# kris927b/TextBlaster

Measured on AMD Instinct MI355X. Metric: documents/sec through full C4+Gopher+langID pipeline at 1/2/4/8 MI355X, higher is better.
Workload: dtype bf16

## Files before the change

### csrc/common/docproc.h

```cpp
#pragma once
#include <type_traits>

#include "devplan.h"
#include "hash.h"
#include "langid.h"
#include "par.h"
#include "uax29.h"
#include "ucd.h"

namespace tb {

enum : int {
  PH_START = 0, PH_DECODE, PH_DICT, PH_PREFIX_HASH, PH_WORDS, PH_LINES, PH_GQ, PH_GR_LINES, PH_GR_WORDS,
  PH_GR_TOP, PH_GR_DUP, PH_FW, PH_LID, PH_GR_DUP_WALK, PH_GR_DUP_CANON, PH_GR_TOP_CANON,
  PH_C4_LOREM = 16, PH_C4_DECODE, PH_C4_LINES, PH_C4_CITE, PH_C4_WORDS, PH_C4_CODES, PH_C4_JOIN, PH_C4_SENT,
  PH_GR_NL = 24, PH_GR_LINE_DUP, PH_GR_WH, PH_GR_WCANON, PH_GQ_WORDS, PH_GQ_BYTES, PH_RUST_LINES,
  kPhaseSlots = 32
};

enum : uint32_t {
  DOC_OK = 0,
  DOC_NEEDS_CPU = 1,
  DOC_OVERFLOW = 2,
};
// ... 1246 lines not shown
    x.par.single([&]() {
      ex->rs = rs; ex->rl = rl; ex->prs = prs; ex->off = off; ex->ph = ph;
      ex->NR = NR; ex->NPR = NPR; ex->tcs = tcs; ex->tce = tce;
      ex->lines_valid = split_lines ? 1u : 0u;
    });
  }
  x.stamp(PH_GR_LINES);
  x.par.single([&]() {
    r[0] = span;
    r[1] = NPR + 1;
    r[2] = para_dup;
    r[3] = para_dup_b;
    r[4] = NR + 1;
    r[5] = line_dup;
    r[6] = line_dup_b;
  });
  const uint32_t W = w.n;
  const bool ngrams = ds.n_top + ds.n_dup > 0;
  if constexpr (P::kWaves == 1) {
    if (ngrams && W >= kWave16) {
      x.set_flag(DOC_NEEDS_CPU);
      return;
    }
  }
  uint32_t* wid = nullptr;
  uint32_t* WL = nullptr;
  uint64_t* K = nullptr;
  uint64_t* PB = nullptr;
  if (ngrams && pre && pre->wready) {
    wid = pre->wid;
    WL = pre->wl;
    K = pre->wk;
    PB = pre->wpb;
  } else if (ngrams) {
    const uint64_t tab_bytes = 6ull * W + 64;
    wid = ex ? x.template alloc<uint32_t>(W + 1) : x.template alloc_hot_keep<uint32_t>(W + 1, tab_bytes);
    WL = ex ? x.template alloc<uint32_t>(W + 1) : x.template alloc_hot_keep<uint32_t>(W + 1, tab_bytes);
    K = ex ? x.template alloc<uint64_t>(W + 1) : x.template alloc_hot_keep<uint64_t>(W + 1, tab_bytes);
    PB = ex ? x.template alloc<uint64_t>(W + 1) : x.template alloc_hot_keep<uint64_t>(W + 1, tab_bytes);
    const bool early = P::kWaves == 1 && release_props && ex != nullptr;
    const auto mw = x.mark();
    uint64_t* wh = early ? x.template alloc_hot<uint64_t>(W + 1) : x.template alloc_hot_hi<uint64_t>(W + 1);
    if (x.overflow) return;
    x.par.for_n(W, [&](uint32_t k) { wh[k] = span_hash8(x, ph, w.bs[k], w.be[k]); });
    x.par.sync();
    if (early) x.release_hi();
    x.stamp(PH_GR_WH);
    canonicalize(
        x, W, [&](uint32_t k) { return dev_key(wh[k], w.be[k] - w.bs[k]); },
        [&](uint32_t i, uint32_t j) { return bytes_eq<P>(b, w.bs[i], w.be[i], w.bs[j], w.be[j]); }, wid);
    x.stamp(PH_GR_WCANON);
    const uint32_t totl = x.par.template scan<uint32_t>(
        W, 0u, [](uint32_t a, uint32_t c2) { return a + c2; },
        [&](uint32_t k) { return w.be[k] - w.bs[k]; }, [&](uint32_t k, uint32_t e) { WL[k] = e; });
    x.par.single([&]() { WL[W] = totl; });
    x.par.sync();
    x.par.for_n(W + 1, [&](uint32_t k) { PB[k] = x.powb(WL[k]); });
    const uint64_t ktot = x.par.template scan<uint64_t>(
        W, 0ull, [](uint64_t a, uint64_t c2) { return a + c2; },
        [&](uint32_t j) { return wh[j] * x.ipowb(WL[j + 1]); }, [&](uint32_t k, uint64_t e) { K[k] = e; });
    x.par.single([&]() { K[W] = ktot; });
    x.par.sync();
    x.reset(mw);
    if (x.overflow) return;
  }
  x.stamp(PH_GR_WORDS);
  if (release_props) x.release_hi();
  if (ngrams) {
    const DupGrams dg{wid, WL, K, PB, w.bs, w.be, b};
// ... 1415 lines not shown
```

### csrc/hip/kernels.hip

```cpp
#include <hip/hip_runtime.h>
#include <algorithm>
#include <cstdlib>
#include <string>

#include "../common/docproc.h"
#include "../common/gate.h"
#include "../common/badwords.h"

using namespace tb;

namespace {

constexpr uint32_t kMaxLdsPerDoc = 160 * 1024;
constexpr uint32_t kMaxLdsPerBlk = 128 * 1024;

struct DevTables {
  const uint16_t* s1;
  const uint32_t* s2;
  const uint16_t* l1;
  const int32_t* l2;
};

extern __shared__ __attribute__((aligned(16))) char g_lds_arena[];

// ... 146 lines not shown
    x.prof = nullptr;
    x.lds = lds_bytes ? (char*)g_lds_arena : nullptr;
    x.lcap = lds_bytes;
    x.lused = 0;
    x.ucd = UcdView{tabs.s1, tabs.s2, tabs.l1, tabs.l2};
    x.pw = pw;
    x.pw_n = pw_n;
    x.ipw = pw ? pw + pw_n + 1 : nullptr;
    const uint64_t region = (e.free_cap / (uint64_t)n_tasks) & ~255ull;
    x.scr = e.free_base + (uint64_t)t * region;
    x.cap = region;
    x.used = 0;
    x.flag = flags + doc;
    x.par.xs = g_block_xs;
    int64_t* r = rec + (int64_t)ds.rec_prefix * ndocs + (int64_t)doc * ds.width;
    if (t < ds.n_dup) gr_dup_one_order(x, ds, t, e, r);
    else if (t < ds.n_dup + ds.n_top) gr_top_one_order(x, ds, t - ds.n_dup, e, r);
    else if (t < ds.n_dup + ds.n_top + 2) gr_lines_split(x, t - ds.n_dup - ds.n_top, e, r);
    if (x.overflow) x.set_flag(DOC_NEEDS_CPU | DOC_OVERFLOW);
    __syncthreads();
  }
}

constexpr int kNgWaves = 4;

template <uint32_t MAXW>
struct NgShared {
  static_assert(MAXW % 64 == 0, "whole waves of grams");
  static constexpr uint32_t kMaxW = MAXW;
  static constexpr uint32_t kCap = MAXW + MAXW / 2 + 4;
  static constexpr uint32_t kSW = (MAXW + 31) / 32 + 1;
  static constexpr uint32_t kBW = MAXW / 2;
  static_assert(2 * kBW <= kCap && (kBW & (kBW - 1)) == 0, "bitmaps fit the table space");
  static constexpr uint32_t kDupBytes = 4 * kCap + 3 * 2 * MAXW + 4 * 2 * ((kSW + 3) & ~3u);
  static constexpr uint32_t kTopBytes = 4 * kCap + 2 * MAXW + 4 * MAXW;
  static constexpr uint32_t kRegion = ((kDupBytes > kTopBytes ? kDupBytes : kTopBytes) + 15) & ~15u;
  uint64_t K[MAXW + 1];
  uint64_t PB[MAXW + 1];
  uint16_t wid[MAXW + 1];
  uint16_t WL[MAXW + 1];
  uint4 region[kNgWaves][kRegion / 16];
};

__device__ __forceinline__ bool ng_fits(const GrExport& e, uint32_t hi) {
  return e.W <= hi && e.WL[e.W] <= 0xFFFFu;
}

__device__ __forceinline__ uint32_t ng_home(uint64_t k, uint32_t capn) {
  return (uint32_t)(((k & 0xFFFFFFFFull) * capn) >> 32);
}

template <class NS, class KeyF>
__device__ __forceinline__ uint32_t ng_candidates(uint32_t G, uint32_t lane, uint32_t* once, uint32_t* twice,
                                                  uint16_t* hbuf, uint16_t* list, KeyF&& key) {
  constexpr uint32_t kMask = NS::kBW * 32u - 1u;
  static_assert(kMask <= 0xFFFFu, "bit index in 16 bits");
#pragma unroll 1
  for (uint32_t p = lane; p < G; p += 64) {
    const uint32_t h = (uint32_t)(key(p) >> 20) & kMask;
    hbuf[p] = (uint16_t)h;
    const uint32_t bit = 1u << (h & 31u);
    if (atomicOr(&once[h >> 5], bit) & bit) atomicOr(&twice[h >> 5], bit);
  }
  __builtin_amdgcn_wave_barrier();
  const uint64_t lt = lane ? (~0ull >> (64 - lane)) : 0ull;
  uint32_t nc = 0;
#pragma unroll 1
  for (uint32_t base = 0; base < G; base += 64) {
    const uint32_t p = base + lane;
    bool c = false;
    if (p < G) {
      const uint32_t h = hbuf[p];
      c = (twice[h >> 5] >> (h & 31u)) & 1u;
    }
    const uint64_t m = __ballot(c);
    if (c) list[nc + (uint32_t)__popcll(m & lt)] = (uint16_t)p;
    nc += (uint32_t)__popcll(m);
  }
  __builtin_amdgcn_wave_barrier();
  return nc;
}

__device__ __attribute__((noinline)) bool ng_dup_eq_bytes(const GrExport* ep, uint32_t p, uint32_t q, uint32_t n) {
  const DupGrams dg{ep->wid, ep->WL, ep->K, ep->PB, ep->bs, ep->be, ep->b};
  return dg.eq(p, q, n);
}
template <class NS>
__device__ __forceinline__ bool ng_dup_eq(const NS& S, const GrExport* ep, uint32_t p, uint32_t q, uint32_t n) {
  if ((uint32_t)(S.WL[p + n] - S.WL[p]) != (uint32_t)(S.WL[q + n] - S.WL[q])) return false;
  uint32_t dw = 0;
  for (uint32_t k = 0; k < n; ++k) dw |= (uint32_t)(S.wid[p + k] ^ S.wid[q + k]);
  if (dw == 0) return true;
  return ng_dup_eq_bytes(ep, p, q, n);
}

template <class NS>
__device__ __forceinline__ int64_t ng_dup_order(NS& S, const GrExport* ep, uint32_t W, uint32_t n, uint32_t lane,
                                                uint4* region, bool prof, uint64_t& c_canon, uint64_t& c_walk) {
  const uint64_t t0 = prof ? __builtin_amdgcn_s_memtime() : 0;
  const uint32_t G = W - n + 1;
  const uint32_t SW = (G + 31) / 32 + 1;
  const uint32_t SWa = (SW + 3u) & ~3u;
  uint32_t* tab = (uint32_t*)region;
  uint16_t* gc = (uint16_t*)(tab + NS::kCap);
  uint16_t* list = gc + NS::kMaxW;
  uint16_t* gsl = list + NS::kMaxW;
  uint32_t* sn = (uint32_t*)(gsl + NS::kMaxW);
  uint32_t* R = sn + SWa;
  for (uint32_t i = lane; i < 2 * NS::kBW; i += 64) tab[i] = 0;
  for (uint32_t i = lane; i < 2 * SWa; i += 64) sn[i] = 0;
  __builtin_amdgcn_wave_barrier();
  auto key = [&](uint32_t p) {
    return dev_key(S.PB[p + n] * (S.K[p + n] - S.K[p]), (uint32_t)(S.WL[p + n] - S.WL[p]));
  };
  const uint32_t nc = ng_candidates<NS>(G, lane, tab, tab + NS::kBW, gc, list, key);
  if (nc < 2) {
    if (prof) c_canon += __builtin_amdgcn_s_memtime() - t0;
    return 0;
  }
  const uint32_t capn = nc + (nc >> 1) + 2;
  for (uint32_t i = lane; i < capn; i += 64) tab[i] = 0;
  __builtin_amdgcn_wave_barrier();
#pragma unroll 1
  for (uint32_t c = lane; c < nc; c += 64) {
    const uint32_t p = list[c];
    const uint64_t k = key(p);
    const uint32_t fp = (uint32_t)(k >> 48);
    const uint32_t mine = (fp << 16) | (c + 1);
    uint32_t sl = ng_home(k, capn);
    while (true) {
      uint32_t cur = tab[sl];
      if (cur == 0) {
        cur = atomicCAS(&tab[sl], 0u, mine);
        if (cur == 0) break;
      }
      if ((cur >> 16) == fp && ng_dup_eq(S, ep, p, list[(cur & 0xFFFFu) - 1u], n)) {
        if ((cur & 0xFFFFu) > c + 1u) atomicMin(&tab[sl], mine);
        break;
      }
      if (++sl == capn) sl = 0;
    }
    gsl[c] = (uint16_t)sl;
  }
  __builtin_amdgcn_wave_barrier();
#pragma unroll 1
  for (uint32_t c = lane; c < nc; c += 64) {
    const uint32_t g = (tab[gsl[c]] & 0xFFFFu) - 1u;
    const uint32_t p = list[c];
    gc[p] = (uint16_t)g;
    if (g != c) {
// ... 45 lines not shown
        A &= A - 1;
      }
    }
    if ((fv >> lane) & 1ull) atomicOr(&sn[g >> 5], 1u << (g & 31));
    uint32_t add = ((cnt >> lane) & 1ull) ? l : 0u;
    for (int o = 32; o > 0; o >>= 1) add += (uint32_t)__shfl_xor((int)add, o);
    rep += add;
    __builtin_amdgcn_wave_barrier();
    idx = next;
  }
  if (prof) c_walk += __builtin_amdgcn_s_memtime() - t1;
  return rep;
}

template <class NS>
__device__ __forceinline__ int64_t ng_top_order(NS& S, uint32_t W, uint32_t n, uint32_t lane, uint4* region) {
  const uint32_t G = W - n + 1;
  uint32_t* tab = (uint32_t*)region;
  uint16_t* list = (uint16_t*)(tab + NS::kCap);
  uint32_t* cnt = (uint32_t*)(list + NS::kMaxW);
  for (uint32_t i = lane; i < 2 * NS::kBW; i += 64) tab[i] = 0;
  __builtin_amdgcn_wave_barrier();
  auto key = [&](uint32_t p) {
    uint64_t h = (uint64_t)n << 56;
    for (uint32_t k = 0; k < n; ++k) h = (h ^ S.wid[p + k]) * 0x9E3779B97F4A7C15ull + k;
    return mix64(h);
  };
  const uint32_t nc = ng_candidates<NS>(G, lane, tab, tab + NS::kBW, (uint16_t*)cnt, list, key);
  if (nc < 2) return 0;
  const uint32_t capn = nc + (nc >> 1) + 2;
  for (uint32_t i = lane; i < capn; i += 64) tab[i] = 0;
  __builtin_amdgcn_wave_barrier();
#pragma unroll 1
  for (uint32_t c = lane; c < nc; c += 64) {
    const uint32_t p = list[c];
    const uint64_t k = key(p);
    const uint32_t fp = (uint32_t)(k >> 48);
    const uint32_t mine = (fp << 16) | (c + 1);
    uint32_t sl = ng_home(k, capn);
    while (true) {
      uint32_t cur = tab[sl];
      if (cur == 0) {
        cur = atomicCAS(&tab[sl], 0u, mine);
        if (cur == 0) break;
      }
      if ((cur >> 16) == fp) {
        const uint32_t qc = (cur & 0xFFFFu) - 1u;
        const uint32_t q = list[qc];
        uint32_t dw = 0;
        for (uint32_t k2 = 0; k2 < n; ++k2) dw |= (uint32_t)(S.wid[p + k2] ^ S.wid[q + k2]);
        if (dw == 0) {
          if (qc > c) atomicMin(&tab[sl], mine);
          break;
        }
      }
      if (++sl == capn) sl = 0;
    }
    cnt[c] = sl << 16;
  }
  __builtin_amdgcn_wave_barrier();
// ... 10 lines not shown
    mx = v > mx ? v : mx;
  }
  if (mx <= 1) return 0;
  uint32_t ml = 0;
  for (uint32_t c = lane; c < nc; c += 64) {
    if ((cnt[c] & 0xFFFFu) != mx) continue;
    const uint32_t p = list[c];
    const uint32_t len = (uint32_t)(S.WL[p + n] - S.WL[p]) + n - 1;
    ml = len > ml ? len : ml;
  }
  for (int o = 32; o > 0; o >>= 1) {
    const uint32_t w = (uint32_t)__shfl_xor((int)ml, o);
    ml = w > ml ? w : ml;
  }
  return (int64_t)ml * (int64_t)mx;
}

#ifndef TB_NG_WPE
#define TB_NG_WPE 8
#endif
struct NgRest {
  uint32_t count;
  uint32_t cursor;
  uint32_t pad[2];
};
__host__ __device__ inline NgRest* ng_rest(const GrExport* ex, int32_t n_docs) {
  return (NgRest*)((char*)ex + (size_t)n_docs * sizeof(GrExport));
}

template <uint32_t MAXW, bool kProf>
__global__ __launch_bounds__(64 * kNgWaves) __attribute__((amdgpu_waves_per_eu(TB_NG_WPE, 8))) void k_gr_ngrams(
    const DevStage* __restrict__ stage, int32_t gr_step, const int32_t* __restrict__ perm, int32_t ndocs,
    const GrExport* __restrict__ ex, int32_t k0, NgRest* rest, int64_t* rec, uint64_t* prof) {
  __shared__ NgShared<MAXW> S;
  const int k = k0 + (int)blockIdx.x;
  const int doc = perm[k];
  if (doc >= ndocs) return;
  const GrExport& e = ex[k];
  if (!e.valid) return;
  const uint32_t W = e.W;
  const uint32_t tid = threadIdx.x, lane = tid & 63, wv = tid >> 6;
  if (!ng_fits(e, MAXW)) {
    if (tid == 0) ((uint32_t*)(rest + 1))[atomicAdd(&rest->count, 1u)] = (uint32_t)k;
    return;
  }
  const DevStep& ds = stage->steps[gr_step];
  int64_t* r = rec + (int64_t)ds.rec_prefix * ndocs + (int64_t)doc * ds.width;
  const int nt = ds.n_dup + ds.n_top;
  uint64_t* pf = kProf ? prof + (size_t)doc * kPhaseSlots : nullptr;
  const uint64_t t0 = kProf ? __builtin_amdgcn_s_memtime() : 0;
  for (uint32_t i = tid; i <= W; i += 64 * kNgWaves) {
    S.K[i] = e.K[i];
    S.PB[i] = e.PB[i];
    S.WL[i] = (uint16_t)e.WL[i];
    S.wid[i] = i < W ? (uint16_t)e.wid[i] : (uint16_t)0;
  }
  __syncthreads();
  if (kProf && tid == 0) atomicAdd((unsigned long long*)&pf[PH_GR_DUP], (unsigned long long)(__builtin_amdgcn_s_memtime() - t0));
  uint64_t c_canon = 0, c_walk = 0, c_top = 0;
  for (int t = (int)wv; t < nt; t += kNgWaves) {
    int64_t v = 0;
    if (t < ds.n_dup) {
      const uint32_t n = (uint32_t)ds.dup_n[t];
      if (n > 0 && W >= n) v = ng_dup_order(S, ex + k, W, n, lane, S.region[wv], kProf, c_canon, c_walk);
    } else {
      const uint32_t n = (uint32_t)ds.top_n[t - ds.n_dup];
      const uint64_t ts = kProf ? __builtin_amdgcn_s_memtime() : 0;
      if (n > 0 && W >= n) v = ng_top_order(S, W, n, lane, S.region[wv]);
      if (kProf) c_top += __builtin_amdgcn_s_memtime() - ts;
    }
    if (lane == 0) r[rec_gr_fixed() + (t < ds.n_dup ? ds.n_top + t : t - ds.n_dup)] = v;
  }
  if (kProf && lane == 0) {
    atomicAdd((unsigned long long*)&pf[PH_GR_DUP_CANON], (unsigned long long)c_canon);
    atomicAdd((unsigned long long*)&pf[PH_GR_DUP_WALK], (unsigned long long)c_walk);
    atomicAdd((unsigned long long*)&pf[PH_GR_TOP_CANON], (unsigned long long)c_top);
  }
}

__global__ __launch_bounds__(64) void k_gr_ngrams_rest(
    const DevStage* __restrict__ stage, int32_t gr_step, const int32_t* __restrict__ perm, int32_t ndocs,
    const GrExport* __restrict__ ex, NgRest* rest, const uint64_t* __restrict__ pw, uint32_t pw_n, DevTables tabs,
    int64_t* rec, uint32_t* flags) {
  const DevStep& ds = stage->steps[gr_step];
  const int nt = ds.n_dup + ds.n_top;
  const uint32_t total = __hip_atomic_load(&rest->count, __ATOMIC_RELAXED, __HIP_MEMORY_SCOPE_AGENT) * (uint32_t)nt;
  const uint32_t* pos = (const uint32_t*)(rest + 1);
  while (true) {
    uint32_t task = 0;
    if (threadIdx.x == 0) task = atomicAdd(&rest->cursor, 1u);
    task = (uint32_t)__builtin_amdgcn_readfirstlane((int)task);
    if (task >= total) break;
    const int k = (int)pos[task / (uint32_t)nt], t = (int)(task % (uint32_t)nt);
    const int doc = perm[k];
    const GrExport e = ex[k];
    int64_t* r = rec + (int64_t)ds.rec_prefix * ndocs + (int64_t)doc * ds.width;
    DocCtx<WavePar> x;
    x.prof = nullptr;
    x.lds = nullptr;
    x.lcap = 0;
    x.lused = 0;
    x.ucd = UcdView{tabs.s1, tabs.s2, tabs.l1, tabs.l2};
    x.pw = pw;
    x.pw_n = pw_n;
    x.ipw = pw ? pw + pw_n + 1 : nullptr;
    const uint64_t region = (e.free_cap / (uint64_t)nt) & ~255ull;
    x.scr = e.free_base + (uint64_t)t * region;
    x.cap = region;
    x.used = 0;
    x.flag = flags + doc;
    if (t < ds.n_dup) gr_dup_one_order(x, ds, t, e, r);
    else gr_top_one_order(x, ds, t - ds.n_dup, e, r);
    if (x.overflow) x.set_flag(DOC_NEEDS_CPU | DOC_OVERFLOW);
  }
}

__global__ __launch_bounds__(64) __attribute__((amdgpu_waves_per_eu(8, 8))) void k_gr_split_wave(
    const DevStage* __restrict__ stage, int32_t gr_step, const int32_t* __restrict__ perm, int32_t n_tasks,
// ... 3 lines not shown
  const int doc = perm[k];
  if (doc >= ndocs) return;
  const GrExport e = ex[k];
  if (!e.valid) return;
  DocCtx<WavePar> x;
  x.prof = nullptr;
  x.lds = lds_bytes ? (char*)g_lds_arena : nullptr;
  x.lcap = lds_bytes;
  x.lused = 0;
  x.ucd = UcdView{tabs.s1, tabs.s2, tabs.l1, tabs.l2};
  x.pw = pw;
  x.pw_n = pw_n;
  x.ipw = pw ? pw + pw_n + 1 : nullptr;
  const uint64_t region = (e.free_cap / (uint64_t)n_tasks) & ~255ull;
  x.scr = e.free_base + (uint64_t)t * region;
  x.cap = region;
  x.used = 0;
  x.flag = flags + doc;
  const DevStep& ds = stage->steps[gr_step];
  int64_t* r = rec + (int64_t)ds.rec_prefix * ndocs + (int64_t)doc * ds.width;
  if (t < ds.n_dup) gr_dup_one_order(x, ds, t, e, r);
  else if (t < ds.n_dup + ds.n_top) gr_top_one_order(x, ds, t - ds.n_dup, e, r);
  if (x.overflow) x.set_flag(DOC_NEEDS_CPU | DOC_OVERFLOW);
}

__device__ __forceinline__ int lid_top(uint64_t m) { return 63 - __clzll((long long)m); }

constexpr int kLidTile = 16;
constexpr int kLidWaves = 8;
typedef __bf16 bf16x8 __attribute__((ext_vector_type(8)));
typedef float f32x4 __attribute__((ext_vector_type(4)));

__device__ __forceinline__ void lid_row_swar(const uint8_t* __restrict__ Eb, uint32_t g, uint32_t* p) {
  const uint4 w = *(const uint4*)(Eb + (size_t)g * kLidRowDim);
  const uint32_t v[4] = {w.x, w.y, w.z, w.w};
#pragma unroll
  for (int q = 0; q < 4; ++q) {
    p[2 * q] += v[q] & 0x00FF00FFu;
    p[2 * q + 1] += (v[q] >> 8) & 0x00FF00FFu;
  }
}

constexpr int kLidSyms = 32;
constexpr int kLidPairs = kLidSyms * kLidSyms;
constexpr uint32_t kLidSymMiss = 32;
constexpr int kLidAuxBytes = kLidPairs * 32 + kLidRowDim;
// ... 946 lines not shown
  if (lds_bytes > 65536)
    (void)hipFuncSetAttribute((const void*)kern, hipFuncAttributeMaxDynamicSharedMemorySize, (int)lds_bytes);
  hipLaunchKernelGGL(kern, dim3(nblocks), dim3(64), lds_bytes, stream, (const DevPlan*)plan,
                     (const DevStage*)stage, d->bytes, d->off, d->perm, d->ndocs, w->scratch, w->scratch_off, tb->pw,
                     tb->pw_n, tb->ucd, w->rec, w->flags, lds_bytes, w->prof, d->dead, line_stats, (GrExport*)gr_export,
                     dict ? *dict : DictIn{});
  return (int)hipGetLastError();
}

int tb_gr_split_wave(hipStream_t stream, const void* stage, int32_t gr_step, const TbDocs* d, int32_t n_tasks,
                     const void* gr_export, const TbWork* w, const TbTables* tb, int32_t block, int32_t n_big) {
  const int32_t* perm = d->perm;
  const int32_t n_docs = d->n_launch, ndocs = d->ndocs;
  const DevTables& t = tb->ucd;
  const uint64_t* pw = tb->pw;
  const uint32_t pw_n = tb->pw_n, lds_bytes = w->lds_bytes;
  int64_t* rec = w->rec;
  uint32_t* flags = w->flags;
  uint64_t* prof = w->prof;
  if (n_docs <= 0 || n_tasks <= 0) return 0;
  if (!perm || !gr_export || gr_step < 0 || gr_step >= kMaxStageSteps || n_tasks > 2 * kMaxNgramEntries ||
      lds_bytes > kMaxLdsPerDoc || n_big < 0 || n_big > n_docs)
    return (int)hipErrorInvalidValue;
  const GrExport* ex = (const GrExport*)gr_export;
  const int32_t n_wave = block ? n_big : n_docs;
  if (n_wave > 0) {
    if (lds_bytes > 65536)
      (void)hipFuncSetAttribute((const void*)k_gr_split_wave, hipFuncAttributeMaxDynamicSharedMemorySize,
                                (int)lds_bytes);
    hipLaunchKernelGGL(k_gr_split_wave, dim3((uint32_t)n_wave * (uint32_t)n_tasks), dim3(64), lds_bytes, stream,
                       (const DevStage*)stage, gr_step, perm, n_tasks, ndocs, ex, pw, pw_n, t, rec, flags, lds_bytes);
  }
  if (block && n_docs > n_big) {
    NgRest* rest = ng_rest(ex, n_docs);
    if (prof)
      hipLaunchKernelGGL((k_gr_ngrams<256, true>), dim3((uint32_t)(n_docs - n_big)), dim3(64 * kNgWaves), 0, stream,
                         (const DevStage*)stage, gr_step, perm, ndocs, ex, n_big, rest, rec, prof);
    else
      hipLaunchKernelGGL((k_gr_ngrams<256, false>), dim3((uint32_t)(n_docs - n_big)), dim3(64 * kNgWaves), 0,
                         stream, (const DevStage*)stage, gr_step, perm, ndocs, ex, n_big, rest, rec, nullptr);
    hipLaunchKernelGGL(k_gr_ngrams_rest, dim3(512), dim3(64), 0, stream, (const DevStage*)stage, gr_step, perm,
                       ndocs, ex, rest, pw, pw_n, t, rec, flags);
  }
  return (int)hipGetLastError();
}

int tb_stage_analyze_blk(hipStream_t stream, const void* plan, const void* stage, const TbDocs* d, const TbWork* w,
                         const TbTables* tb, void* gr_export, int32_t n_split, uint32_t split_bytes,
                         uint32_t* line_stats, const void* pre, const DictIn* dict) {
  const int32_t nblocks = d->n_launch;
  const uint32_t lds_bytes = w->lds_bytes;
  if (nblocks <= 0) return 0;
  if (!d->perm || lds_bytes > kMaxLdsPerBlk || n_split < 0 || n_split > nblocks) return (int)hipErrorInvalidValue;
  auto kern = pre ? k_stage_analyze_blk_pre : k_stage_analyze_blk;
  if (lds_bytes > 65536)
    (void)hipFuncSetAttribute((const void*)kern, hipFuncAttributeMaxDynamicSharedMemorySize, (int)lds_bytes);
  hipLaunchKernelGGL(kern, dim3(nblocks), dim3(kBlockThreads), lds_bytes, stream, (const DevPlan*)plan,
                     (const DevStage*)stage, d->bytes, d->off, d->perm, d->ndocs, w->scratch, w->scratch_off, tb->pw,
                     tb->pw_n, tb->ucd, w->rec, w->flags, lds_bytes, w->prof, d->dead, (GrExport*)gr_export, n_split,
                     split_bytes, line_stats, (const PreDoc*)pre, pre ? nblocks : 0, dict ? *dict : DictIn{});
  return (int)hipGetLastError();
}

int tb_gr_dup_split(hipStream_t stream, const void* stage, int32_t gr_step, const TbDocs* d, int32_t n_tasks,
                    const void* gr_export, const TbWork* w, const TbTables* tb, uint32_t* cursor) {
  const int32_t n_split = d->n_launch;
// ... 177 lines not shown
    const int rc = tb_scan_strided_i64(stream, lanes + j, 4, ndocs, sc + (int64_t)j * ndocs);
    if (rc) return rc;
  }
  if (cap / (ndocs > 0 ? ndocs : 1) > 8192)
    hipLaunchKernelGGL(k_compact<256>, dim3(ndocs), dim3(kCompactThreads), 0, stream, status, fver, vt, ndocs, sc, out, cap, out_off, rows,
                     err);
  else
    hipLaunchKernelGGL(k_compact<64>, dim3((ndocs + 3) / 4), dim3(kCompactThreads), 0, stream, status, fver, vt, ndocs, sc, out, cap, out_off, rows,
                     err);
  return (int)hipGetLastError();
}

size_t tb_sizeof_resolve() { return sizeof(DevResolve); }


int tb_pow_table(hipStream_t stream, uint64_t* pw, uint32_t n) {
  hipLaunchKernelGGL(k_pow_table, dim3((n + 256) / 256), dim3(256), 0, stream, pw, n);
  return (int)hipGetLastError();
}

int tb_phase_slots() { return kPhaseSlots; }
int tb_stage_waves() { return TB_STAGE_WPE; }

int tb_abi_version() { return 25; }
size_t tb_sizeof_plan() { return sizeof(DevPlan); }
size_t tb_sizeof_stage() { return sizeof(DevStage); }
size_t tb_sizeof_c4() { return sizeof(DevC4); }

}
```

### textblaster_amd/ops/kernels.py

```python
from __future__ import annotations

import ctypes
from typing import Optional

import numpy as np

from ..errors import DeviceError

_P = ctypes.c_void_p
_I32 = ctypes.c_int32
_U32 = ctypes.c_uint32
_I64 = ctypes.c_int64
_SZ = ctypes.c_size_t

ABI_VERSION = 25


def _ptr(t) -> Optional[int]:
    return None if t is None else t.data_ptr()


class Tables(ctypes.Structure):
    _fields_ = [("s1", _P), ("s2", _P), ("l1", _P), ("l2", _P), ("pw", _P), ("pw_n", _U32)]


class Docs(ctypes.Structure):
    _fields_ = [("bytes", _P), ("off", _P), ("perm", _P), ("dead", _P), ("n_launch", _I32), ("ndocs", _I32)]

    @classmethod
    def of(cls, bytes_, off, perm, n_launch, ndocs, dead=None):
        if perm is not None and perm.numel() < n_launch:
            raise DeviceError("launch: the permutation is shorter than the launch")
        return cls(_ptr(bytes_), _ptr(off), _ptr(perm), _ptr(dead), int(n_launch), int(ndocs))


class Work(ctypes.Structure):
    _fields_ = [("scratch", _P), ("scratch_off", _P), ("rec", _P), ("flags", _P), ("prof", _P), ("lds_bytes", _U32)]

# ... 148 lines not shown
        if n > self._pw_n:
            from . import hiprt

            cap = max(n, 1 << 16)
            cap = 1 << (cap - 1).bit_length()
            self._pw = hiprt.empty(2 * cap + 2, np.int64)
            _check(self.lib.tb_pow_table(self.stream(), self._pw.data_ptr(), cap), "tb_pow_table")
            hiprt.current_stream().synchronize()
            self._pw_n = cap
        return self._pw, self._pw_n

    def tables(self, pw, pw_n) -> Tables:
        return Tables(*[t.data_ptr() for t in self.tabs], pw.data_ptr(), pw_n)

    def stage_analyze(self, plan, stage, docs: Docs, work: Work, tables: Tables, line_stats=None, gr_export=None,
                      dict_in: Optional[DictIn] = None):
        if gr_export is not None and gr_export.nbytes < max(docs.n_launch, 0) * self.sizeof_gr_export:
            raise DeviceError("stage_analyze: export buffer too small")
        rc = self.lib.tb_stage_analyze(self.stream(), plan.data_ptr(), stage.data_ptr(), docs, work, tables,
                                       _ptr(line_stats), _ptr(gr_export), dict_in)
        _check(rc, "tb_stage_analyze")

    def gr_export_wave_bytes(self, n_docs: int) -> int:
        return n_docs * self.sizeof_gr_export + 16 + 4 * n_docs

    def gr_split_wave(self, stage, gr_step, docs: Docs, n_tasks, gr_export, work: Work, tables: Tables, block=True,
                      n_big=0):
        if not 0 <= n_big <= docs.n_launch:
            raise DeviceError("gr_split_wave: n_big out of range")
        if gr_export.nbytes < self.gr_export_wave_bytes(docs.n_launch):
            raise DeviceError("gr_split_wave: operand shapes")
        rc = self.lib.tb_gr_split_wave(self.stream(), stage.data_ptr(), gr_step, docs, n_tasks, gr_export.data_ptr(),
                                       work, tables, 1 if block else 0, int(n_big))
        _check(rc, "tb_gr_split_wave")

    def stage_analyze_blk(self, plan, stage, docs: Docs, work: Work, tables: Tables, gr_export=None, n_split=0,
                          split_bytes=0, line_stats=None, pre=None, dict_in: Optional[DictIn] = None):
        if gr_export is not None and gr_export.nbytes < n_split * self.sizeof_gr_export:
            raise DeviceError("stage_analyze_blk: export buffer too small")
        if not 0 <= n_split <= docs.n_launch:
            raise DeviceError("stage_analyze_blk: n_split out of range")
        rc = self.lib.tb_stage_analyze_blk(self.stream(), plan.data_ptr(), stage.data_ptr(), docs, work, tables,
                                           _ptr(gr_export), n_split if gr_export is not None else 0, split_bytes,
                                           _ptr(line_stats), _ptr(pre), dict_in)
        _check(rc, "tb_stage_analyze_blk")

    def pre_decode(self, docs: Docs, pre, tiles_max, cnt, tables: Tables):
# ... 115 lines not shown
```

Before: 13.73 million.

## Build word ids and gram hashes in LDS inside n-gram kernel

For exported documents the analyze stage no longer computes word hashes, canonical word ids, prefix sums and power tables. It now exports only word spans and defers that work to the n-gram kernel. That kernel builds a rotate-xor prefix hash, canonical ids via an LDS hash table, and 16-bit length prefixes directly in shared memory from a staged copy of the text. Gram keys move to 32-bit hashes, and byte equality now walks spans directly. Large documents get a dedicated 512-word kernel plus a persistent 1024-word list kernel. A fallback k_gr_words kernel builds the old global tables for misfits. The default ngram wave count also drops from four to three. The aim is to remove global-memory table traffic and 64-bit multiply hashing, at the cost of much more kernel complexity and new hash-collision behaviour.

```diff
diff --git a/csrc/common/docproc.h b/csrc/common/docproc.h
--- a/csrc/common/docproc.h
+++ b/csrc/common/docproc.h
@@ -1292,6 +1292,22 @@
       x.set_flag(DOC_NEEDS_CPU);
       return;
     }
+    if (ngrams && ex) {
+      const uint64_t base = (x.used + 255) & ~255ull;
+      x.par.single([&]() {
+        for (int t = 0; t < ds.n_top + ds.n_dup; ++t) r[rec_gr_fixed() + t] = 0;
+        ex->bs = w.bs; ex->be = w.be;
+        ex->b = b_export ? b_export : b;
+        ex->free_base = x.scr + base;
+        ex->free_cap = x.cap > base ? x.cap - base : 0;
+        ex->W = W;
+        ex->valid = x.overflow ? 0u : 1u;
+      });
+      x.par.sync();
+      x.stamp(PH_GR_WORDS);
+      x.reset(mark);
+      return;
+    }
   }
   uint32_t* wid = nullptr;
   uint32_t* WL = nullptr;
@@ -1308,13 +1324,11 @@
     WL = ex ? x.template alloc<uint32_t>(W + 1) : x.template alloc_hot_keep<uint32_t>(W + 1, tab_bytes);
     K = ex ? x.template alloc<uint64_t>(W + 1) : x.template alloc_hot_keep<uint64_t>(W + 1, tab_bytes);
     PB = ex ? x.template alloc<uint64_t>(W + 1) : x.template alloc_hot_keep<uint64_t>(W + 1, tab_bytes);
-    const bool early = P::kWaves == 1 && release_props && ex != nullptr;
     const auto mw = x.mark();
-    uint64_t* wh = early ? x.template alloc_hot<uint64_t>(W + 1) : x.template alloc_hot_hi<uint64_t>(W + 1);
+    uint64_t* wh = x.template alloc_hot_hi<uint64_t>(W + 1);
     if (x.overflow) return;
     x.par.for_n(W, [&](uint32_t k) { wh[k] = span_hash8(x, ph, w.bs[k], w.be[k]); });
     x.par.sync();
-    if (early) x.release_hi();
     x.stamp(PH_GR_WH);
     canonicalize(
         x, W, [&](uint32_t k) { return dev_key(wh[k], w.be[k] - w.bs[k]); },
diff --git a/csrc/hip/kernels.hip b/csrc/hip/kernels.hip
--- a/csrc/hip/kernels.hip
+++ b/csrc/hip/kernels.hip
@@ -192,12 +192,30 @@
   }
 }
 
-constexpr int kNgWaves = 4;
-
-template <uint32_t MAXW>
+#ifndef TB_NG_WAVES
+#define TB_NG_WAVES 3
+#endif
+constexpr int kNgWaves = TB_NG_WAVES;
+constexpr uint32_t kNgTextBytes = 4096;
+constexpr uint32_t kNgTextSmall = 2048;
+
+template <uint32_t MAXW, uint32_t TEXTB>
+struct NgBuild {
+  static constexpr uint32_t kTextW = TEXTB / 4 + 2;
+  static constexpr uint32_t kCap = MAXW + MAXW / 2 + 4;
+  uint64_t T[256];
+  uint64_t wkey[MAXW];
+  uint32_t txt[kTextW];
+  uint32_t tab[kCap];
+  uint16_t ws[MAXW];
+  uint16_t slot[MAXW];
+};
+
+template <uint32_t MAXW, uint32_t TEXTB = (MAXW <= 256 ? kNgTextSmall : kNgTextBytes)>
 struct NgShared {
   static_assert(MAXW % 64 == 0, "whole waves of grams");
   static constexpr uint32_t kMaxW = MAXW;
+  static constexpr uint32_t kTextBytes = TEXTB;
   static constexpr uint32_t kCap = MAXW + MAXW / 2 + 4;
   static constexpr uint32_t kSW = (MAXW + 31) / 32 + 1;
   static constexpr uint32_t kBW = MAXW / 2;
@@ -205,19 +223,123 @@
   static constexpr uint32_t kDupBytes = 4 * kCap + 3 * 2 * MAXW + 4 * 2 * ((kSW + 3) & ~3u);
   static constexpr uint32_t kTopBytes = 4 * kCap + 2 * MAXW + 4 * MAXW;
   static constexpr uint32_t kRegion = ((kDupBytes > kTopBytes ? kDupBytes : kTopBytes) + 15) & ~15u;
-  uint64_t K[MAXW + 1];
-  uint64_t PB[MAXW + 1];
+  static_assert(sizeof(NgBuild<MAXW, TEXTB>) <= kNgWaves * kRegion, "the build's arrays fit the regions");
+  static_assert(kCap <= 0xFFFFu && TEXTB + 8 <= 0xFFFFu, "16-bit slots, word starts and byte prefixes");
+  uint64_t Q[MAXW + 1];
   uint16_t wid[MAXW + 1];
   uint16_t WL[MAXW + 1];
   uint4 region[kNgWaves][kRegion / 16];
 };
 
-__device__ __forceinline__ bool ng_fits(const GrExport& e, uint32_t hi) {
-  return e.W <= hi && e.WL[e.W] <= 0xFFFFu;
-}
-
-__device__ __forceinline__ uint32_t ng_home(uint64_t k, uint32_t capn) {
-  return (uint32_t)(((k & 0xFFFFFFFFull) * capn) >> 32);
+__device__ __forceinline__ uint32_t ng_home(uint32_t k, uint32_t capn) {
+  return (uint32_t)(((uint64_t)k * capn) >> 32);
+}
+
+__device__ __forceinline__ uint32_t ng_mix32(uint32_t x) {
+  x ^= x >> 16;
+  x *= 0x85EBCA6Bu;
+  x ^= x >> 13;
+  x *= 0xC2B2AE35u;
+  x ^= x >> 16;
+  return x;
+}
+__device__ __forceinline__ uint64_t ng_rotl(uint64_t x, uint32_t r) { return (x << (r & 63u)) | (x >> ((64u - r) & 63u)); }
+__device__ __forceinline__ uint64_t ng_rotr(uint64_t x, uint32_t r) { return (x >> (r & 63u)) | (x << ((64u - r) & 63u)); }
+
+constexpr uint32_t kNgRot = 5;
+
+template <class NS>
+__device__ __forceinline__ void ng_build(NS& S, const GrExport& e, uint32_t W, uint32_t bs0, uint32_t tid) {
+  using NB = NgBuild<NS::kMaxW, NS::kTextBytes>;
+  NB& B = *(NB*)&S.region[0][0];
+  constexpr uint32_t NT = 64 * kNgWaves;
+  const uint32_t lane = tid & 63;
+  const uint8_t* g0 = e.b + bs0;
+  const uintptr_t a0 = (uintptr_t)g0 & ~(uintptr_t)3;
+  const uint32_t head = (uint32_t)((uintptr_t)g0 - a0);
+  const uint32_t nd = (head + (e.be[W - 1] - bs0) + 3) >> 2;
+  const uint32_t* src = (const uint32_t*)a0;
+  for (uint32_t i = tid; i < nd; i += NT) B.txt[i] = src[i];
+  for (uint32_t c = tid; c < 256; c += NT)
+    B.T[c] = ((uint64_t)ng_mix32(2 * c + 1) << 32) | ng_mix32(2 * c + 0x9E3779B2u);
+  const uint32_t capn = W + (W >> 1) + 2;
+  for (uint32_t i = tid; i < capn; i += NT) B.tab[i] = 0;
+  __syncthreads();
+  const uint8_t* t8 = (const uint8_t*)B.txt;
+#pragma unroll 1
+  for (uint32_t k = tid; k < W; k += NT) {
+    const uint32_t s = e.bs[k] - bs0 + head, len = e.be[k] - e.bs[k];
+    uint64_t h = 0, pk = 0;
+    for (uint32_t i = 0; i < len; ++i) {
+      const uint32_t c = t8[s + i];
+      h = ng_rotl(h, kNgRot) ^ B.T[c];
+      if (i < 8) pk |= (uint64_t)c << (8 * i);
+    }
+    B.ws[k] = (uint16_t)s;
+    B.wkey[k] = len <= 8 ? pk : h;
+    S.Q[k + 1] = h;
+    S.WL[k + 1] = (uint16_t)len;
+  }
+  __syncthreads();
+  if (tid < 64) {
+    uint32_t cl = 0;
+    uint64_t cq = 0;
+    if (lane == 0) { S.WL[0] = 0; S.Q[0] = 0; }
+#pragma unroll 1
+    for (uint32_t base = 0; base < W; base += 64) {
+      const uint32_t k = base + lane;
+      uint32_t l = k < W ? (uint32_t)S.WL[k + 1] : 0u;
+      for (int o = 1; o < 64; o <<= 1) {
+        const uint32_t v = (uint32_t)__shfl_up((int)l, o);
+        if ((int)lane >= o) l += v;
+      }
+      l += cl;
+      uint64_t q = k < W ? ng_rotr(S.Q[k + 1], kNgRot * l) : 0ull;
+      for (int o = 1; o < 64; o <<= 1) {
+        const uint32_t lo = (uint32_t)__shfl_up((int)(uint32_t)q, o), hi = (uint32_t)__shfl_up((int)(uint32_t)(q >> 32), o);
+        if ((int)lane >= o) q ^= ((uint64_t)hi << 32) | lo;
+      }
+      q ^= cq;
+      if (k < W) { S.WL[k + 1] = (uint16_t)l; S.Q[k + 1] = q; }
+      cl = (uint32_t)__shfl((int)l, 63);
+      cq = ((uint64_t)(uint32_t)__shfl((int)(uint32_t)(q >> 32), 63) << 32) | (uint32_t)__shfl((int)(uint32_t)q, 63);
+    }
+  }
+  __syncthreads();
+#pragma unroll 1
+  for (uint32_t k = tid; k < W; k += NT) {
+    const uint64_t key = B.wkey[k];
+    const uint32_t len = (uint32_t)(S.WL[k + 1] - S.WL[k]);
+    const uint32_t hk = ng_mix32((uint32_t)key + (uint32_t)(key >> 32) * 0x9E3779B1u + len);
+    const uint32_t fp = hk & 0xFFFFu;
+    const uint32_t mine = (fp << 16) | (k + 1);
+    uint32_t sl = ng_home(hk, capn);
+    while (true) {
+      uint32_t cur = B.tab[sl];
+      if (cur == 0) {
+        cur = atomicCAS(&B.tab[sl], 0u, mine);
+        if (cur == 0) break;
+      }
+      if ((cur >> 16) == fp) {
+        const uint32_t q = (cur & 0xFFFFu) - 1u;
+        bool same = B.wkey[q] == key && (uint32_t)(S.WL[q + 1] - S.WL[q]) == len;
+        if (same && len > 8) {
+          const uint32_t sa = B.ws[k], sb = B.ws[q];
+          for (uint32_t i = 8; i < len && same; ++i) same = t8[sa + i] == t8[sb + i];
+          for (uint32_t i = 0; i < 8 && same; ++i) same = t8[sa + i] == t8[sb + i];
+        }
+        if (same) {
+          if (q > k) atomicMin(&B.tab[sl], mine);
+          break;
+        }
+      }
+      if (++sl == capn) sl = 0;
+    }
+    B.slot[k] = (uint16_t)sl;
+  }
+  __syncthreads();
+  for (uint32_t k = tid; k <= W; k += NT) S.wid[k] = k < W ? (uint16_t)((B.tab[B.slot[k]] & 0xFFFFu) - 1u) : (uint16_t)0;
+  __syncthreads();
 }
 
 template <class NS, class KeyF>
@@ -227,7 +349,7 @@
   static_assert(kMask <= 0xFFFFu, "bit index in 16 bits");
 #pragma unroll 1
   for (uint32_t p = lane; p < G; p += 64) {
-    const uint32_t h = (uint32_t)(key(p) >> 20) & kMask;
+    const uint32_t h = key(p) & kMask;
     hbuf[p] = (uint16_t)h;
     const uint32_t bit = 1u << (h & 31u);
     if (atomicOr(&once[h >> 5], bit) & bit) atomicOr(&twice[h >> 5], bit);
@@ -251,17 +373,28 @@
   return nc;
 }
 
-__device__ __attribute__((noinline)) bool ng_dup_eq_bytes(const GrExport* ep, uint32_t p, uint32_t q, uint32_t n) {
-  const DupGrams dg{ep->wid, ep->WL, ep->K, ep->PB, ep->bs, ep->be, ep->b};
-  return dg.eq(p, q, n);
+__device__ __attribute__((noinline)) bool ng_dup_eq_bytes(const GrExport* ep, uint32_t p, uint32_t q, uint32_t L) {
+  const uint32_t* bs = ep->bs;
+  const uint32_t* be = ep->be;
+  const uint8_t* b = ep->b;
+  uint32_t wp = p, wq = q, bp = bs[p], bq = bs[q];
+  for (uint32_t i = 0; i < L; ++i) {
+    while (bp == be[wp]) { ++wp; bp = bs[wp]; }
+    while (bq == be[wq]) { ++wq; bq = bs[wq]; }
+    if (b[bp] != b[bq]) return false;
+    ++bp;
+    ++bq;
+  }
+  return true;
 }
 template <class NS>
 __device__ __forceinline__ bool ng_dup_eq(const NS& S, const GrExport* ep, uint32_t p, uint32_t q, uint32_t n) {
-  if ((uint32_t)(S.WL[p + n] - S.WL[p]) != (uint32_t)(S.WL[q + n] - S.WL[q])) return false;
+  const uint32_t L = (uint32_t)(S.WL[p + n] - S.WL[p]);
+  if (L != (uint32_t)(S.WL[q + n] - S.WL[q])) return false;
   uint32_t dw = 0;
   for (uint32_t k = 0; k < n; ++k) dw |= (uint32_t)(S.wid[p + k] ^ S.wid[q + k]);
   if (dw == 0) return true;
-  return ng_dup_eq_bytes(ep, p, q, n);
+  return ng_dup_eq_bytes(ep, p, q, L);
 }
 
 template <class NS>
@@ -281,7 +414,9 @@
   for (uint32_t i = lane; i < 2 * SWa; i += 64) sn[i] = 0;
   __builtin_amdgcn_wave_barrier();
   auto key = [&](uint32_t p) {
-    return dev_key(S.PB[p + n] * (S.K[p + n] - S.K[p]), (uint32_t)(S.WL[p + n] - S.WL[p]));
+    const uint32_t e = S.WL[p + n];
+    const uint64_t h = ng_rotl(S.Q[p + n] ^ S.Q[p], kNgRot * e);
+    return ng_mix32((uint32_t)h + (uint32_t)(h >> 32) * 0x9E3779B1u + (e - (uint32_t)S.WL[p]));
   };
   const uint32_t nc = ng_candidates<NS>(G, lane, tab, tab + NS::kBW, gc, list, key);
   if (nc < 2) {
@@ -294,8 +429,8 @@
 #pragma unroll 1
   for (uint32_t c = lane; c < nc; c += 64) {
     const uint32_t p = list[c];
-    const uint64_t k = key(p);
-    const uint32_t fp = (uint32_t)(k >> 48);
+    const uint32_t k = key(p);
+    const uint32_t fp = (k >> 12) & 0xFFFFu;
     const uint32_t mine = (fp << 16) | (c + 1);
     uint32_t sl = ng_home(k, capn);
     while (true) {
@@ -387,9 +522,9 @@
   for (uint32_t i = lane; i < 2 * NS::kBW; i += 64) tab[i] = 0;
   __builtin_amdgcn_wave_barrier();
   auto key = [&](uint32_t p) {
-    uint64_t h = (uint64_t)n << 56;
-    for (uint32_t k = 0; k < n; ++k) h = (h ^ S.wid[p + k]) * 0x9E3779B97F4A7C15ull + k;
-    return mix64(h);
+    uint32_t h = n;
+    for (uint32_t k = 0; k < n; ++k) h = (h ^ S.wid[p + k]) * 0x9E3779B1u + k;
+    return ng_mix32(h);
   };
   const uint32_t nc = ng_candidates<NS>(G, lane, tab, tab + NS::kBW, (uint16_t*)cnt, list, key);
   if (nc < 2) return 0;
@@ -399,8 +534,8 @@
 #pragma unroll 1
   for (uint32_t c = lane; c < nc; c += 64) {
     const uint32_t p = list[c];
-    const uint64_t k = key(p);
-    const uint32_t fp = (uint32_t)(k >> 48);
+    const uint32_t k = key(p);
+    const uint32_t fp = (k >> 12) & 0xFFFFu;
     const uint32_t mine = (fp << 16) | (c + 1);
     uint32_t sl = ng_home(k, capn);
     while (true) {
@@ -457,40 +592,33 @@
 struct NgRest {
   uint32_t count;
   uint32_t cursor;
-  uint32_t pad[2];
+  uint32_t count_big;
+  uint32_t cursor_big;
+  uint32_t cursor_words;
+  uint32_t pad[3];
 };
 __host__ __device__ inline NgRest* ng_rest(const GrExport* ex, int32_t n_docs) {
   return (NgRest*)((char*)ex + (size_t)n_docs * sizeof(GrExport));
 }
 
 template <uint32_t MAXW, bool kProf>
-__global__ __launch_bounds__(64 * kNgWaves) __attribute__((amdgpu_waves_per_eu(TB_NG_WPE, 8))) void k_gr_ngrams(
-    const DevStage* __restrict__ stage, int32_t gr_step, const int32_t* __restrict__ perm, int32_t ndocs,
-    const GrExport* __restrict__ ex, int32_t k0, NgRest* rest, int64_t* rec, uint64_t* prof) {
-  __shared__ NgShared<MAXW> S;
-  const int k = k0 + (int)blockIdx.x;
+__device__ __forceinline__ bool ng_document(NgShared<MAXW>& S, const DevStage* __restrict__ stage, int32_t gr_step,
+                                            const int32_t* __restrict__ perm, int32_t ndocs,
+                                            const GrExport* __restrict__ ex, int k, int64_t* rec, uint64_t* prof) {
   const int doc = perm[k];
-  if (doc >= ndocs) return;
+  if (doc >= ndocs) return true;
   const GrExport& e = ex[k];
-  if (!e.valid) return;
+  if (!e.valid) return true;
   const uint32_t W = e.W;
   const uint32_t tid = threadIdx.x, lane = tid & 63, wv = tid >> 6;
-  if (!ng_fits(e, MAXW)) {
-    if (tid == 0) ((uint32_t*)(rest + 1))[atomicAdd(&rest->count, 1u)] = (uint32_t)k;
-    return;
-  }
+  const uint32_t bs0 = W ? e.bs[0] : 0u;
+  if (W > MAXW || (W && e.be[W - 1] - bs0 > NgShared<MAXW>::kTextBytes)) return false;
   const DevStep& ds = stage->steps[gr_step];
   int64_t* r = rec + (int64_t)ds.rec_prefix * ndocs + (int64_t)doc * ds.width;
   const int nt = ds.n_dup + ds.n_top;
   uint64_t* pf = kProf ? prof + (size_t)doc * kPhaseSlots : nullptr;
   const uint64_t t0 = kProf ? __builtin_amdgcn_s_memtime() : 0;
-  for (uint32_t i = tid; i <= W; i += 64 * kNgWaves) {
-    S.K[i] = e.K[i];
-    S.PB[i] = e.PB[i];
-    S.WL[i] = (uint16_t)e.WL[i];
-    S.wid[i] = i < W ? (uint16_t)e.wid[i] : (uint16_t)0;
-  }
-  __syncthreads();
+  if (W) ng_build(S, e, W, bs0, tid);
   if (kProf && tid == 0) atomicAdd((unsigned long long*)&pf[PH_GR_DUP], (unsigned long long)(__builtin_amdgcn_s_memtime() - t0));
   uint64_t c_canon = 0, c_walk = 0, c_top = 0;
   for (int t = (int)wv; t < nt; t += kNgWaves) {
@@ -510,6 +638,132 @@
     atomicAdd((unsigned long long*)&pf[PH_GR_DUP_CANON], (unsigned long long)c_canon);
     atomicAdd((unsigned long long*)&pf[PH_GR_DUP_WALK], (unsigned long long)c_walk);
     atomicAdd((unsigned long long*)&pf[PH_GR_TOP_CANON], (unsigned long long)c_top);
+  }
+  return true;
+}
+
+template <uint32_t MAXW, bool kProf>
+__global__ __launch_bounds__(64 * kNgWaves) __attribute__((amdgpu_waves_per_eu(TB_NG_WPE, 8))) void k_gr_ngrams(
+    const DevStage* __restrict__ stage, int32_t gr_step, const int32_t* __restrict__ perm, int32_t ndocs,
+    const GrExport* __restrict__ ex, int32_t k0, int32_t n_docs, NgRest* rest, int64_t* rec, uint64_t* prof) {
+  __shared__ NgShared<MAXW> S;
+  const int k = k0 + (int)blockIdx.x;
+  if (!ng_document<MAXW, kProf>(S, stage, gr_step, perm, ndocs, ex, k, rec, prof) && threadIdx.x == 0)
+    ((uint32_t*)(rest + 1))[n_docs + atomicAdd(&rest->count_big, 1u)] = (uint32_t)k;
+}
+
+template <uint32_t MAXW, bool kProf>
+__global__ __launch_bounds__(64 * kNgWaves) __attribute__((amdgpu_waves_per_eu(TB_NG_WPE, 8))) void k_gr_ngrams_big(
+    const DevStage* __restrict__ stage, int32_t gr_step, const int32_t* __restrict__ perm, int32_t ndocs,
+    const GrExport* __restrict__ ex, int32_t k0, int32_t n_docs, NgRest* rest, int64_t* rec, uint64_t* prof) {
+  __shared__ NgShared<MAXW> S;
+  const int k = k0 + (int)blockIdx.x;
+  if (!ng_document<MAXW, kProf>(S, stage, gr_step, perm, ndocs, ex, k, rec, prof) && threadIdx.x == 0)
+    ((uint32_t*)(rest + 1))[n_docs + atomicAdd(&rest->count_big, 1u)] = (uint32_t)k;
+}
+
+template <uint32_t MAXW, bool kProf>
+__global__ __launch_bounds__(64 * kNgWaves) __attribute__((amdgpu_waves_per_eu(TB_NG_WPE, 8))) void k_gr_ngrams_list(
+    const DevStage* __restrict__ stage, int32_t gr_step, const int32_t* __restrict__ perm, int32_t ndocs,
+    const GrExport* __restrict__ ex, int32_t n_docs, NgRest* rest, int64_t* rec, uint64_t* prof) {
+  __shared__ NgShared<MAXW> S;
+  __shared__ uint32_t s_next;
+  const uint32_t total = __hip_atomic_load(&rest->count_big, __ATOMIC_RELAXED, __HIP_MEMORY_SCOPE_AGENT);
+  uint32_t* pos = (uint32_t*)(rest + 1);
+  constexpr uint32_t kNone = 0xFFFFFFFFu;
+  uint32_t misfit = kNone;
+  while (true) {
+    if (threadIdx.x == 0) {
+      if (misfit != kNone) pos[atomicAdd(&rest->count, 1u)] = misfit;
+      s_next = atomicAdd(&rest->cursor_big, 1u);
+    }
+    __syncthreads();
+    const uint32_t i = s_next;
+    __syncthreads();
+    if (i >= total) break;
+    const int k = (int)pos[n_docs + i];
+    misfit = ng_document<MAXW, kProf>(S, stage, gr_step, perm, ndocs, ex, k, rec, prof) ? kNone : (uint32_t)k;
+  }
+}
+
+__global__ __launch_bounds__(64) void k_gr_words(const int32_t* __restrict__ perm, int32_t ndocs, GrExport* ex,
+                                                 NgRest* rest, int32_t n_all, const uint64_t* __restrict__ pw,
+                                                 uint32_t pw_n, DevTables tabs, uint32_t* flags) {
+  const uint32_t total =
+      n_all > 0 ? 0u : __hip_atomic_load(&rest->count, __ATOMIC_RELAXED, __HIP_MEMORY_SCOPE_AGENT);
+  const uint32_t* pos = (const uint32_t*)(rest + 1);
+  while (true) {
+    int k = (int)blockIdx.x;
+    if (n_all <= 0) {
+      uint32_t i = 0;
+      if (threadIdx.x == 0) i = atomicAdd(&rest->cursor_words, 1u);
+      i = (uint32_t)__builtin_amdgcn_readfirstlane((int)i);
+      if (i >= total) break;
+      k = (int)pos[i];
+    }
+    const int doc = perm[k];
+    GrExport& e = ex[k];
+    if (doc < ndocs && e.valid) {
+      const uint32_t W = e.W;
+      const uint32_t* bs = e.bs;
+      const uint32_t* be = e.be;
+      const uint8_t* b = e.b;
+      DocCtx<WavePar> x;
+      x.prof = nullptr;
+      x.lds = nullptr;
+      x.lcap = 0;
+      x.lused = 0;
+      x.ucd = UcdView{tabs.s1, tabs.s2, tabs.l1, tabs.l2};
+      x.pw = pw;
+      x.pw_n = pw_n;
+      x.ipw = pw ? pw + pw_n + 1 : nullptr;
+      x.scr = e.free_base;
+      x.cap = e.free_cap;
+      x.used = 0;
+      x.flag = flags + doc;
+      uint32_t* wid = x.template alloc<uint32_t>(W + 1);
+      uint32_t* WL = x.template alloc<uint32_t>(W + 1);
+      uint64_t* K = x.template alloc<uint64_t>(W + 1);
+      uint64_t* PB = x.template alloc<uint64_t>(W + 1);
+      const uint64_t keep = x.used;
+      uint64_t* wh = x.template alloc<uint64_t>(W + 1);
+      if (!x.overflow) {
+        x.par.for_n(W, [&](uint32_t j) {
+          uint64_t h = 0;
+          for (uint32_t i = bs[j]; i < be[j]; ++i) h = hash_push(h, b[i]);
+          wh[j] = h;
+        });
+        x.par.sync();
+        canonicalize(
+            x, W, [&](uint32_t j) { return dev_key(wh[j], be[j] - bs[j]); },
+            [&](uint32_t i, uint32_t j) { return bytes_eq<WavePar>(b, bs[i], be[i], bs[j], be[j]); }, wid);
+      }
+      if (!x.overflow) {
+        const uint32_t totl = x.par.template scan<uint32_t>(
+            W, 0u, [](uint32_t a, uint32_t c2) { return a + c2; }, [&](uint32_t j) { return be[j] - bs[j]; },
+            [&](uint32_t j, uint32_t v) { WL[j] = v; });
+        x.par.single([&]() { WL[W] = totl; });
+        x.par.sync();
+        x.par.for_n(W + 1, [&](uint32_t j) { PB[j] = x.powb(WL[j]); });
+        const uint64_t ktot = x.par.template scan<uint64_t>(
+            W, 0ull, [](uint64_t a, uint64_t c2) { return a + c2; },
+            [&](uint32_t j) { return wh[j] * x.ipowb(WL[j + 1]); }, [&](uint32_t j, uint64_t v) { K[j] = v; });
+        x.par.single([&]() { K[W] = ktot; });
+        x.par.sync();
+      }
+      if (x.overflow) x.set_flag(DOC_NEEDS_CPU | DOC_OVERFLOW);
+      const uint64_t base = (keep + 255) & ~255ull;
+      const bool ok = !x.overflow && base <= e.free_cap;
+      x.par.single([&]() {
+        e.wid = wid; e.WL = WL; e.K = K; e.PB = PB;
+        if (ok) {
+          e.free_base += base;
+          e.free_cap -= base;
+        }
+        e.valid = ok ? 1u : 0u;
+      });
+    }
+    if (n_all > 0) break;
   }
 }
 
@@ -529,6 +783,7 @@
     const int k = (int)pos[task / (uint32_t)nt], t = (int)(task % (uint32_t)nt);
     const int doc = perm[k];
     const GrExport e = ex[k];
+    if (!e.valid) continue;
     int64_t* r = rec + (int64_t)ds.rec_prefix * ndocs + (int64_t)doc * ds.width;
     DocCtx<WavePar> x;
     x.prof = nullptr;
@@ -578,6 +833,21 @@
   if (t < ds.n_dup) gr_dup_one_order(x, ds, t, e, r);
   else if (t < ds.n_dup + ds.n_top) gr_top_one_order(x, ds, t - ds.n_dup, e, r);
   if (x.overflow) x.set_flag(DOC_NEEDS_CPU | DOC_OVERFLOW);
+}
+
+template <bool kProf>
+static void launch_gr_ngrams(hipStream_t stream, const DevStage* stage, int32_t gr_step, const int32_t* perm,
+                             int32_t ndocs, const GrExport* ex, int32_t n_docs, int32_t n_big, NgRest* rest,
+                             int64_t* rec, uint64_t* prof, uint32_t list_grid) {
+  const dim3 nt(64 * kNgWaves);
+  if (n_big > 0)
+    hipLaunchKernelGGL((k_gr_ngrams_big<512, kProf>), dim3((uint32_t)n_big), nt, 0, stream, stage, gr_step, perm, ndocs,
+                       ex, 0, n_docs, rest, rec, prof);
+  if (n_docs > n_big)
+    hipLaunchKernelGGL((k_gr_ngrams<256, kProf>), dim3((uint32_t)(n_docs - n_big)), nt, 0, stream, stage, gr_step,
+                       perm, ndocs, ex, n_big, n_docs, rest, rec, prof);
+  hipLaunchKernelGGL((k_gr_ngrams_list<1024, kProf>), dim3(list_grid), nt, 0, stream, stage, gr_step,
+                     perm, ndocs, ex, n_docs, rest, rec, prof);
 }
 
 __device__ __forceinline__ int lid_top(uint64_t m) { return 63 - __clzll((long long)m); }
@@ -1570,26 +1840,27 @@
   if (!perm || !gr_export || gr_step < 0 || gr_step >= kMaxStageSteps || n_tasks > 2 * kMaxNgramEntries ||
       lds_bytes > kMaxLdsPerDoc || n_big < 0 || n_big > n_docs)
     return (int)hipErrorInvalidValue;
-  const GrExport* ex = (const GrExport*)gr_export;
-  const int32_t n_wave = block ? n_big : n_docs;
-  if (n_wave > 0) {
+  GrExport* ex = (GrExport*)gr_export;
+  NgRest* rest = ng_rest(ex, n_docs);
+  if (!block) {
     if (lds_bytes > 65536)
       (void)hipFuncSetAttribute((const void*)k_gr_split_wave, hipFuncAttributeMaxDynamicSharedMemorySize,
                                 (int)lds_bytes);
-    hipLaunchKernelGGL(k_gr_split_wave, dim3((uint32_t)n_wave * (uint32_t)n_tasks), dim3(64), lds_bytes, stream,
+    hipLaunchKernelGGL(k_gr_words, dim3((uint32_t)n_docs), dim3(64), 0, stream, perm, ndocs, ex, rest, n_docs, pw, pw_n,
+                       t, flags);
+    hipLaunchKernelGGL(k_gr_split_wave, dim3((uint32_t)n_docs * (uint32_t)n_tasks), dim3(64), lds_bytes, stream,
                        (const DevStage*)stage, gr_step, perm, n_tasks, ndocs, ex, pw, pw_n, t, rec, flags, lds_bytes);
-  }
-  if (block && n_docs > n_big) {
-    NgRest* rest = ng_rest(ex, n_docs);
-    if (prof)
-      hipLaunchKernelGGL((k_gr_ngrams<256, true>), dim3((uint32_t)(n_docs - n_big)), dim3(64 * kNgWaves), 0, stream,
-                         (const DevStage*)stage, gr_step, perm, ndocs, ex, n_big, rest, rec, prof);
-    else
-      hipLaunchKernelGGL((k_gr_ngrams<256, false>), dim3((uint32_t)(n_docs - n_big)), dim3(64 * kNgWaves), 0,
-                         stream, (const DevStage*)stage, gr_step, perm, ndocs, ex, n_big, rest, rec, nullptr);
-    hipLaunchKernelGGL(k_gr_ngrams_rest, dim3(512), dim3(64), 0, stream, (const DevStage*)stage, gr_step, perm,
-                       ndocs, ex, rest, pw, pw_n, t, rec, flags);
-  }
+    return (int)hipGetLastError();
+  }
+  const uint32_t list_grid = 3u * (uint32_t)device_cus();
+  if (prof)
+    launch_gr_ngrams<true>(stream, (const DevStage*)stage, gr_step, perm, ndocs, ex, n_docs, n_big, rest, rec, prof, list_grid);
+  else
+    launch_gr_ngrams<false>(stream, (const DevStage*)stage, gr_step, perm, ndocs, ex, n_docs, n_big, rest, rec, nullptr,
+                            list_grid);
+  hipLaunchKernelGGL(k_gr_words, dim3(256), dim3(64), 0, stream, perm, ndocs, ex, rest, 0, pw, pw_n, t, flags);
+  hipLaunchKernelGGL(k_gr_ngrams_rest, dim3(512), dim3(64), 0, stream, (const DevStage*)stage, gr_step, perm, ndocs,
+                     ex, rest, pw, pw_n, t, rec, flags);
   return (int)hipGetLastError();
 }
 
@@ -1813,7 +2084,7 @@
 int tb_phase_slots() { return kPhaseSlots; }
 int tb_stage_waves() { return TB_STAGE_WPE; }
 
-int tb_abi_version() { return 25; }
+int tb_abi_version() { return 26; }
 size_t tb_sizeof_plan() { return sizeof(DevPlan); }
 size_t tb_sizeof_stage() { return sizeof(DevStage); }
 size_t tb_sizeof_c4() { return sizeof(DevC4); }
diff --git a/textblaster_amd/ops/kernels.py b/textblaster_amd/ops/kernels.py
--- a/textblaster_amd/ops/kernels.py
+++ b/textblaster_amd/ops/kernels.py
@@ -13,7 +13,7 @@
 _I64 = ctypes.c_int64
 _SZ = ctypes.c_size_t
 
-ABI_VERSION = 25
+ABI_VERSION = 26
 
 
 def _ptr(t) -> Optional[int]:
@@ -208,7 +208,7 @@
         _check(rc, "tb_stage_analyze")
 
     def gr_export_wave_bytes(self, n_docs: int) -> int:
-        return n_docs * self.sizeof_gr_export + 16 + 4 * n_docs
+        return n_docs * self.sizeof_gr_export + 32 + 8 * n_docs
 
     def gr_split_wave(self, stage, gr_step, docs: Docs, n_tasks, gr_export, work: Work, tables: Tables, block=True,
                       n_big=0):
```

Measured after the change: 14.88 million (median of 6 runs). 1.08x the previous value.
